# niessner/BundleFusion

Hardware: AMD Instinct MI355X
Metric: frames/sec end-to-end (SIFT+SBA+TSDF re-integrate), 640x480 @4mm (higher is better)
Workload: dtype f32

## Files before the change

### bundlefusion_amd/capi.py

```python
import ctypes as C
import os

import numpy as np

_HERE = os.path.dirname(os.path.abspath(__file__))
LIB_PATH = os.environ.get("BF_LIB_PATH") or os.path.join(_HERE, "lib", "libbf_hip.so")


class BFError(RuntimeError):
    pass


if not os.path.exists(LIB_PATH):
    raise ImportError(
        "bundlefusion_amd: %s is missing — build it with `python -c 'import __graft_entry__ as g; g.build()'` "
        "(there is no CPU fallback)" % LIB_PATH)

try:
    import torch
except ImportError:
    pass
lib = C.CDLL(LIB_PATH, mode=C.RTLD_GLOBAL)

SDF_BLOCK_SIZE = 8
# ... 212 lines not shown
            o.d_texels = None; o.wait_event = None
        check(lib.bf_scene_run_batch(self._h, arr, len(ops), C.byref(cam)))

    def garbage_collect(self):
        check(lib.bf_scene_garbage_collect(self._h))

    def compactify(self, cam_to_world, cam):
        check(lib.bf_scene_set_last_rigid_transform_and_compactify(self._h, mat16(cam_to_world), C.byref(cam)))

    def hash_data(self):
        hd = HashData()
        check(lib.bf_scene_get_hash_data(self._h, C.byref(hd)))
        return hd

    def hash_params(self):
        p = HashParams()
        check(lib.bf_scene_get_hash_params(self._h, C.byref(p)))
        return p

    def heap_free_count(self):
        v = C.c_uint32()
        check(lib.bf_scene_get_heap_free_count(self._h, C.byref(v)))
        return v.value

    def num_allocated_blocks(self):
        v = C.c_uint32()
        check(lib.bf_scene_get_num_allocated_blocks(self._h, C.byref(v)))
        return v.value

    def num_integrated_frames(self):
        v = C.c_uint32()
        check(lib.bf_scene_get_num_integrated_frames(self._h, C.byref(v)))
        return v.value

    def debug_hash(self):
        out = (C.c_uint32 * 6)()
        check(lib.bf_scene_debug_hash(self._h, out))
        return dict(occupied=out[0], heap_free=out[1], duplicate_keys=out[2], free_and_allocated=out[3], leaked=out[4],
                    dropped=out[5])

    def find_blocks(self, pos):
        import torch
        out = torch.empty(pos.shape[0], dtype=torch.int32, device=pos.device)
        check(lib.bf_scene_debug_find_blocks(self._h, C.c_void_p(pos.data_ptr()), int(pos.shape[0]), C.c_void_p(out.data_ptr())))
        return out

    def kernel_timing(self, enable):
        check(lib.bf_scene_kernel_timing(self._h, int(enable)))

    def kernel_timing_read(self):
        n, ms = C.c_uint32(), C.c_float()
        check(lib.bf_scene_kernel_timing_read(self._h, C.byref(n), C.byref(ms)))
        return n.value, ms.value

    def kernel_timing_occupied(self):
        v = C.c_uint64(); n = C.c_uint32()
        check(lib.bf_scene_kernel_timing_occupied(self._h, C.byref(v), C.byref(n)))
        return v.value, n.value

    def kernel_timing_blocks(self):
        a = C.c_uint64(); b = C.c_uint64(); c = C.c_uint64(); n = C.c_uint32()
        check(lib.bf_scene_kernel_timing_blocks(self._h, C.byref(a), C.byref(b), C.byref(c), C.byref(n)))
        return a.value, b.value, c.value, n.value

    def kernel_timing_images(self):
        n = C.c_uint32()
# ... 1233 lines not shown
```

### bundlefusion_amd/csrc/tsdf.hip

```cpp
#include <hip/hip_runtime.h>

#include <algorithm>
#include <cmath>
#include <cstdlib>
#include <cstring>
#include <strings.h>
#include <unordered_map>
#include <unordered_set>
#include <vector>

#include "bf_device.h"
#include "bf_internal.h"
#include "../../include/bf_comm.h"

using namespace bf;

namespace {

constexpr int BS = BF_SDF_BLOCK_SIZE;
constexpr int VOX = BS * BS * BS;
constexpr uint32_t NBINS = 256;
constexpr uint32_t BINCAP = 4096;
constexpr uint32_t OVCAP = 4096;
constexpr uint32_t TILE = 1024;
constexpr uint64_t EMPTY64 = ~0ull;
constexpr int KEYLIM = 1 << 20;

struct AllocRec { uint64_t key; int32_t ptr; uint32_t pad; };
struct BinRec { uint64_t key; uint32_t bucket; uint32_t aux; };

enum Stat { ST_DROPPED = 0, ST_ERROR = 1, ST_STUCK = 2, ST_TICKET = 3, ST_COUNT = 4 };
enum ErrBits { ERR_BIN_OVERFLOW = 1, ERR_DEDUPE_FULL = 2, ERR_OV_OVERFLOW = 4, ERR_GC_MISSING = 8, ERR_LIST_FULL = 16 };

struct Dev {
    bf_hash_entry* hash;
    uint32_t* heap;
    uint32_t* heapCounter;
    bf_voxel* vox;
    bf_hash_entry* compact;
    uint32_t* compactSrc;
    int32_t* compactCount;
    AllocRec* allocList;
    AllocRec* allocListAlt;
    uint32_t* allocCount;
    uint32_t* allocSnap;
    uint64_t* dedupe;
    uint32_t dedupeMask;
    BinRec* bins;
    uint32_t* binCount;
    BinRec* overflow;
    uint32_t* overflowCount;
    uint32_t* stuckSlots;
    uint32_t* tileCounts;
    uint32_t* stats;
    unsigned long long* occSum;
};

struct Frame {
    m44 T, Tinv;
    bf_depth_camera_params cam;
    uint32_t numBuckets;
    uint32_t maxChain;
    uint32_t numSDFBlocks;
    float voxelSize;
// ... 1260 lines not shown
    const uint32_t lane = threadIdx.x & 63u;
    const uint32_t wave = __builtin_amdgcn_readfirstlane(blockIdx.x * 4u + (threadIdx.x >> 6)), nWaves = gridDim.x * 4u;
    if (accumulate && wave == 0 && lane == 0) {
        if (MODE == 2) { d.occSum[2] += (unsigned long long)n; d.occSum[0] += (unsigned long long)(uint32_t)d.compactCount[1]; }
        else { d.occSum[0] += (unsigned long long)n; d.occSum[1] += (unsigned long long)n; }
    }
    if (wave >= n) return;
    const __amdgpu_buffer_rsrc_t texRes = __builtin_amdgcn_make_buffer_rsrc(const_cast<uint2*>(tex), 0, (int)(2u * c.bytes), 0x00020000);
    for (uint32_t blk = wave; blk < n; blk += nWaves) {
        const ApxEntry en = apxEntry<MODE>(d, blk);
        const ApxBlock cur = apxBlock<DE, IN>(d, c, in, de, en.e, en.flags, lane);
#pragma unroll 1
        for (int z = 0; z < 8; z += 2) {
            ApxPair pa;
            apxSamples<DE, IN>(c, in, de, cur, z, texRes, pa);
            bool anyA, anyB;
            apxTouched<DE, IN>(c, pa, anyA, anyB);
            const bool ldA = __builtin_amdgcn_ballot_w64(anyA) != 0ull, ldB = __builtin_amdgcn_ballot_w64(anyB) != 0ull;
            if (!ldA && !ldB) continue;
            apxLoadVoxels(cur, z, pa, ldA, ldB);
            apxStageB<DE, IN, RNE>(c, cur, z, pa);
        }
    }
}


__global__ void k_probe_cvt(uint32_t* out) {
    const float v[8] = {0.5f, 1.5f, 2.5f, 2.7f, 254.4f, 300.0f, -3.0f, 3.49f};
    if (threadIdx.x < 8) out[threadIdx.x] = __builtin_amdgcn_cvt_pk_u8_f32(v[threadIdx.x], 1u, 0xAABBCCDDu);
}

#include "tsdf_batch.h"

__global__ __launch_bounds__(256) void k_gc_identify(Dev d, Frame f, uint32_t needMask) {
    __shared__ uint32_t wmax[4];
    const uint32_t n = (uint32_t)d.compactCount[0];
    for (uint32_t blk = blockIdx.x; blk < n; blk += gridDim.x) {
        if (needMask != 0u && (reinterpret_cast<const uint32_t*>(d.compact)[(size_t)blk * 8 + 4] & needMask) == 0u) continue;
        const int4 e = reinterpret_cast<const int4*>(d.compact)[(size_t)blk * 2];
        const bf_voxel* v = d.vox + (size_t)(uint32_t)e.w;
        const uint32_t w0 = (uint32_t)f2i(v[2 * threadIdx.x + 0].weight);
        const uint32_t w1 = (uint32_t)f2i(v[2 * threadIdx.x + 1].weight);
        uint32_t m = wave_max_u(max(w0, w1));
        if ((threadIdx.x & 63) == 0) wmax[threadIdx.x >> 6] = m;
        __syncthreads();
        if (threadIdx.x == 0) {
            m = max(max(wmax[0], wmax[1]), max(wmax[2], wmax[3]));
            if (m == 0) {
                i3 b; b.x = e.x; b.y = e.y; b.z = e.z;
                const uint32_t h = hashPos(f.numBuckets, b);
                const uint32_t bin = (uint32_t)(((uint64_t)h * NBINS) / f.numBuckets);
                const uint32_t pos = atomicAdd(&d.binCount[bin], 1u);
                if (pos < BINCAP) {
                    BinRec r; r.key = packKey(b); r.bucket = h; r.aux = d.compactSrc[blk];
                    d.bins[(size_t)bin * BINCAP + pos] = r;
                } else {
                    atomicOr(&d.stats[ST_ERROR], (uint32_t)ERR_BIN_OVERFLOW);
                }
            }
        }
        __syncthreads();
    }
}

BF_DEV int32_t deleteEntry(const Dev& d, const Frame& f, i3 b, uint32_t h) {
    const uint32_t hp = h * BF_HASH_BUCKET_SIZE;
    const uint32_t total = BF_HASH_BUCKET_SIZE * f.numBuckets;
    uint4* h4 = reinterpret_cast<uint4*>(d.hash);
    for (uint32_t j = 0; j < BF_HASH_BUCKET_SIZE; ++j) {
        const uint32_t i = hp + j;
        const bf_hash_entry c = d.hash[i];
        if (c.pos[0] == b.x && c.pos[1] == b.y && c.pos[2] == b.z && c.ptr != BF_FREE_ENTRY) {
            if (c.offset != 0) {
                const uint32_t next = (i + c.offset) % total;
                h4[(size_t)i * 2] = h4[(size_t)next * 2];
                h4[(size_t)i * 2 + 1] = h4[(size_t)next * 2 + 1];
                h4[(size_t)next * 2] = make_uint4(0, 0, 0, (uint32_t)BF_FREE_ENTRY);
                h4[(size_t)next * 2 + 1] = make_uint4(0, 0, 0, 0);
            } else {
                h4[(size_t)i * 2] = make_uint4(0, 0, 0, (uint32_t)BF_FREE_ENTRY);
                h4[(size_t)i * 2 + 1] = make_uint4(0, 0, 0, 0);
            }
            return c.ptr;
        }
    }
    const uint32_t last = hp + BF_HASH_BUCKET_SIZE - 1;
    bf_hash_entry c = d.hash[last];
    uint32_t prev = last;
    uint32_t i = (last + c.offset) % total;
    for (uint32_t it = 0; it < f.maxChain; ++it) {
        c = d.hash[i];
        if (c.pos[0] == b.x && c.pos[1] == b.y && c.pos[2] == b.z && c.ptr != BF_FREE_ENTRY) {
            h4[(size_t)i * 2] = make_uint4(0, 0, 0, (uint32_t)BF_FREE_ENTRY);
            h4[(size_t)i * 2 + 1] = make_uint4(0, 0, 0, 0);
            d.hash[prev].offset = c.offset;
            return c.ptr;
        }
        if (c.offset == 0) return BF_FREE_ENTRY;
        prev = i;
        i = (last + c.offset) % total;
    }
    return BF_FREE_ENTRY;
}

__global__ __launch_bounds__(1024) void k_gc_delete(Dev d, Frame f) {
    __shared__ SortLds s;
    __shared__ uint32_t scratch[16];
    const uint32_t bin = blockIdx.x;
    const uint32_t n = min(d.binCount[bin], BINCAP);
    if (n == 0) return;
    loadBinSorted(s, d.bins + (size_t)bin * BINCAP, n);
    const uint32_t base = binPrefix(d.binCount, bin, scratch);
    const uint32_t heapC = d.heapCounter[0];
    for (uint32_t idx = threadIdx.x; idx < n; idx += blockDim.x) {
        const uint32_t h = s.bucket[idx];
        if (idx > 0 && s.bucket[idx - 1] == h) continue;
        for (uint32_t k = idx; k < n && s.bucket[k] == h; ++k) {
            const int32_t ptr = deleteEntry(d, f, unpackKey(s.key[k]), h);
            d.allocList[s.aux[k]].ptr = BF_FREE_ENTRY;
            if (ptr == BF_FREE_ENTRY) { atomicOr(&d.stats[ST_ERROR], (uint32_t)ERR_GC_MISSING); s.aux[k] = 0xFFFFFFFFu; continue; }
            d.heap[heapC + 1u + base + k] = (uint32_t)ptr / (uint32_t)VOX;
            s.aux[k] = (uint32_t)ptr;
        }
    }
    __syncthreads();
    for (uint32_t k = 0; k < n; ++k) {
        const uint32_t ptr = s.aux[k];
        if (ptr == 0xFFFFFFFFu) continue;
        uint4* v4 = reinterpret_cast<uint4*>(d.vox + (size_t)ptr);
        for (uint32_t t = threadIdx.x; t < (uint32_t)(VOX * 12 / 16); t += blockDim.x) v4[t] = make_uint4(0, 0, 0, 0);
    }
}

__global__ __launch_bounds__(256) void k_gc_finish(Dev d) {
    __shared__ uint32_t scratch[16];
    const uint32_t D = binPrefix(d.binCount, NBINS, scratch);
    if (threadIdx.x == 0) d.heapCounter[0] += D;
    __syncthreads();
    for (uint32_t b = threadIdx.x; b < NBINS; b += blockDim.x) d.binCount[b] = 0;
}

}

struct bf_scene {
    bf_hash_params params;
    bf_depth_camera_params cam;
    bool haveCam = false;
    Dev d{};
    hipStream_t stream = nullptr;
    uint32_t numIntegrated = 0;
    uint32_t dedupeSize = 0;
    uint32_t gridCompact = 0, gridUpdateCol = 0, gridUpdateColPlain = 0;
    bool forceExactDiv = false;
    bool externalAlloc = false;
    bf_comm* allocComm = nullptr;
    uint32_t allocCap = 0;
    uint8_t *d_allocSend = nullptr, *d_allocRecv = nullptr; uint32_t* d_allocSlots = nullptr;
    uint8_t *d_batchSend = nullptr, *d_batchRecv = nullptr;
    int arith = BF_TSDF_ARITH_FAST;
    int cvtRne = -1;
    uint2* texel[8] = {}; size_t texelPixels = 0;
    int32_t* d_hashDecision = nullptr;
    uint32_t shardLo = 0, shardHi = 0xFFFFFFFFu;
    uint32_t opsTimed = 0;
    uint32_t imagesTimed = 0;
    bool overlap = false;
    hipStream_t prep = nullptr;
    static constexpr int NBMAX = 8;
    int NB = 4;
    bf_hash_entry* cbuf[NBMAX] = {}; uint32_t* csrc[NBMAX] = {}; int32_t* ccnt[NBMAX] = {};
    int cur = 0;
    hipEvent_t evPrep[NBMAX] = {}, evUpd[NBMAX] = {}, evBarrier = nullptr, evTmp = nullptr;
    bool updRecorded[NBMAX] = {};
    bool barrierPending = false;
    hipEvent_t pendingEv = nullptr;
    const uint2* frameTexels = nullptr;
    bool compactStale = false;
    uint32_t gcMask = 0;
    BatchDev bd{};
    bool batchReady = false;
    uint2* btexel[NBMAX][BF_SCENE_BATCH_MAX] = {}; size_t btexelPixels = 0;
    uint32_t updateLds = 0;
    const char* verifyPath = nullptr; bf_voxel* vshadow[2] = {}; VerifyLog* vlog = nullptr; uint32_t vseq = 0;
    bool timing = false;
    std::vector<std::pair<hipEvent_t, hipEvent_t>> events;
    size_t eventsUsed = 0;
    std::vector<void*> allocations;
};

#define BF_TRY_RC(expr) do { int _rc = (expr); if (_rc != BF_OK) return _rc; } while (0)

namespace {

template <class T>
int devAlloc(bf_scene* s, T** p, size_t count) {
    void* q = nullptr;
    hipError_t e = BF_MALLOC(&q, count * sizeof(T));
    if (e != hipSuccess) { set_error("BF_MALLOC(%zu B) failed: %s", count * sizeof(T), hipGetErrorString(e)); return BF_ERR_HIP; }
    s->allocations.push_back(q);
    *p = (T*)q;
    return BF_OK;
}

Frame makeFrame(const bf_scene* s) {
    Frame f;
    memcpy(f.T.e, s->params.m_rigidTransform, 64);
    memcpy(f.Tinv.e, s->params.m_rigidTransformInverse, 64);
    f.cam = s->cam;
    f.numBuckets = s->params.m_hashNumBuckets;
    f.maxChain = s->params.m_hashMaxCollisionLinkedListSize;
// ... 337 lines not shown
    bc.tile0 = (uint32_t)((uint64_t)tiles * rank / world); bc.tile1 = (uint32_t)((uint64_t)tiles * (rank + 1) / world);
    if (bc.tile1 > bc.tile0) hipLaunchKernelGGL(k_batch_march, dim3(div_up(bc.tile1 - bc.tile0, 4), n), dim3(256), 0, ms, dv, s->bd, bc, ma);
    if (s->allocComm) {
        const uint64_t brec = 8 + sizeof(BatchRec) * (uint64_t)s->allocCap;
        hipLaunchKernelGGL(k_batch_pack, dim3(256), dim3(256), 0, ms, dv, s->bd, reinterpret_cast<uint32_t*>(s->d_batchSend), reinterpret_cast<BatchRec*>(s->d_batchSend + 8), s->allocCap);
        hipLaunchKernelGGL(k_batch_pack_finish, dim3(1), dim3(1), 0, ms, s->bd);
        BF_TRY_RC(bf_comm_all_gather(s->allocComm, s->d_batchSend, s->d_batchRecv, brec, ms));
        for (uint32_t r = 0; r < world; ++r) {
            const uint8_t* base = s->d_batchRecv + brec * r;
            hipLaunchKernelGGL(k_batch_ingest, dim3(256), dim3(256), 0, ms, dv, s->bd, reinterpret_cast<const uint32_t*>(base), reinterpret_cast<const BatchRec*>(base + 8), s->allocCap);
        }
    }
    if (s->overlap && s->barrierPending) { BF_HIP_TRY(hipStreamWaitEvent(ps, s->evBarrier, 0)); s->barrierPending = false; }
    hipLaunchKernelGGL(k_batch_bin, dim3(1024), dim3(256), 0, ps, dv, s->bd, bc);
    hipLaunchKernelGGL(k_batch_place, dim3(PLACE_WGS), dim3(256), 0, ps, dv, s->bd, bc, fr);
    if (s->overlap) {
        BF_HIP_TRY(hipEventRecord(s->evPrep[b], ps));
        BF_HIP_TRY(hipStreamWaitEvent(s->stream, s->evPrep[b], 0));
    }
    std::pair<hipEvent_t, hipEvent_t>* ev = nullptr;
    if (s->timing) {
        if (s->eventsUsed == s->events.size()) {
            hipEvent_t e0, e1;
            BF_HIP_TRY(hipEventCreate(&e0));
            BF_HIP_TRY(hipEventCreate(&e1));
            s->events.push_back({e0, e1});
        }
        ev = &s->events[s->eventsUsed++];
        s->opsTimed += opsCount;
        s->imagesTimed += n;
        BF_HIP_TRY(hipEventRecord(ev->first, s->stream));
    }
    const int acc = s->timing ? 1 : 0;
    if (fast) {
        BatchUpdApxArgs ua;
        memset(&ua, 0, sizeof ua);
        ua.nOps = n;
        for (uint32_t k = 0; k < n; ++k) {
            ua.op[k].in = makeApxPose(fin[k]); ua.op[k].de = makeApxPose(fde[k]);
            ua.op[k].tex = ops[k].d_texels ? reinterpret_cast<const uint2*>(ops[k].d_texels) : texelOf[k];
            if (ops[k].data.d_colorData) ua.liveMask |= 3u << (2u * k);
        }
        const ApxCam ac = makeApxCam(fl);
        auto update = [&](const Dev& dd, int accumulate) {
            if (s->cvtRne) hipLaunchKernelGGL((k_update_batch_apx<true>), dim3(s->gridUpdateCol), dim3(256), s->updateLds, s->stream, dd, ac, ua, accumulate);
            else hipLaunchKernelGGL((k_update_batch_apx<false>), dim3(s->gridUpdateCol), dim3(256), s->updateLds, s->stream, dd, ac, ua, accumulate);
        };
        if (s->verifyPath) {
            BF_TRY_RC(verifyBuffers(s));
            hipLaunchKernelGGL(k_verify_copy, dim3(s->gridUpdateCol), dim3(256), 0, s->stream, dv, s->vshadow[0], s->vshadow[1]);
        }
        update(dv, acc);
        if (s->verifyPath) {
            for (int q = 0; q < 2; ++q) { Dev dq = dv; dq.vox = s->vshadow[q]; update(dq, 0); }
            hipLaunchKernelGGL(k_verify_compare, dim3(s->gridUpdateCol), dim3(256), 0, s->stream, dv, s->vshadow[0], s->vshadow[1], s->vlog, s->vseq++, n, s->gridUpdateCol * 4u);
        }
    } else {
        BatchUpdColArgs ua;
        memset(&ua, 0, sizeof ua);
        ua.nOps = n;
        for (uint32_t k = 0; k < n; ++k) {
            ua.op[k].in = makeUpdPose(fin[k]); ua.op[k].de = makeUpdPose(fde[k]);
            ua.op[k].depth = ops[k].data.d_depthData; ua.op[k].color = reinterpret_cast<const uchar4*>(ops[k].data.d_colorData);
        }
        hipLaunchKernelGGL(k_update_batch_col, dim3(s->gridUpdateCol), dim3(256), 0, s->stream, dv, makeUpdCam(fl), ua, acc, s->forceExactDiv ? 1 : 0);
    }
    if (ev) BF_HIP_TRY(hipEventRecord(ev->second, s->stream));
    if (s->overlap) { BF_HIP_TRY(hipEventRecord(s->evUpd[b], s->stream)); s->updRecorded[b] = true; }
    BF_HIP_TRY(hipGetLastError());
    useBuf(s, b);
    s->compactStale = true;
    s->gcMask = (ops[n - 1].kind == 1 ? 2u : 1u) << (2u * (n - 1));
    for (uint32_t k = 0; k < n; ++k) s->numIntegrated += ops[k].kind == 0 ? 1u : ops[k].kind == 1 ? (uint32_t)-1 : 0u;
    return BF_OK;
}

int checkCall(bf_scene* s, const float* T, const bf_depth_camera_data* data, const bf_depth_camera_params* cam,
              const uint32_t* d_bitMask) {
    BF_REQUIRE(s && T && data && cam, "null argument");
    BF_REQUIRE(data->d_depthData, "d_depthData is null");
    BF_REQUIRE(d_bitMask == nullptr, "chunk streaming (d_bitMask) is not supported: it is disabled for BundleFusion");
    BF_REQUIRE(cam->m_imageWidth > 0 && cam->m_imageHeight > 0, "empty image");
    return BF_OK;
}

}

extern "C" {

int bf_scene_create(const bf_hash_params* p, bf_scene** out) {
    BF_REQUIRE(p && out, "null argument");
    BF_REQUIRE(p->m_hashNumBuckets > 0 && p->m_numSDFBlocks > 0, "empty hash / heap");
    BF_REQUIRE(p->m_hashBucketSize == BF_HASH_BUCKET_SIZE, "m_hashBucketSize must be 4 (HASH_BUCKET_SIZE)");
    BF_REQUIRE(p->m_SDFBlockSize == BF_SDF_BLOCK_SIZE, "m_SDFBlockSize must be 8 (SDF_BLOCK_SIZE)");
    BF_REQUIRE((uint64_t)p->m_hashNumBuckets * BF_HASH_BUCKET_SIZE < 0x7FFFFFFFull, "hash too large for 32-bit slot indices");
    BF_REQUIRE((uint64_t)p->m_numSDFBlocks * VOX < 0x7FFFFFFFull, "too many SDF blocks for the reference's int ptr");
    int ndev = 0;
    if (hipGetDeviceCount(&ndev) != hipSuccess || ndev == 0) { set_error("no HIP device visible"); return BF_ERR_NO_DEVICE; }
    bf_scene* s = new bf_scene();
    s->params = *p;
    const size_t numEntries = (size_t)p->m_hashNumBuckets * BF_HASH_BUCKET_SIZE;
    const size_t N = p->m_numSDFBlocks;
    uint32_t ds = 1u << 16;
    while (ds < 2u * NBINS * BINCAP && ds < 4u * N) ds <<= 1;
    s->dedupeSize = ds;
    int rc = BF_OK;
#define A(ptr, cnt) if (rc == BF_OK) rc = devAlloc(s, &(ptr), (cnt))
    A(s->d.hash, numEntries);
    A(s->d.heap, N);
    A(s->d.heapCounter, 1);
    A(s->d.vox, N * VOX);
    for (int b = 0; b < bf_scene::NBMAX; ++b) { A(s->cbuf[b], N); A(s->csrc[b], N); A(s->ccnt[b], 4); }
    A(s->d.occSum, 3);
    A(s->d.allocList, N);
    A(s->d.allocListAlt, N);
    A(s->d.allocCount, 1);
    A(s->d.dedupe, (size_t)ds);
    A(s->d.bins, (size_t)NBINS * BINCAP);
    A(s->d.binCount, NBINS);
    A(s->d.overflow, OVCAP);
    A(s->d.overflowCount, 1);
    A(s->d.stuckSlots, OVCAP);
    A(s->d.tileCounts, N / TILE + 4);
    A(s->d.stats, ST_COUNT);
    A(s->d_hashDecision, 4);
#undef A
    if (rc != BF_OK) { bf_scene_destroy(s); return rc; }
    s->d.dedupeMask = ds - 1;
    useBuf(s, 0);
    {
        int least = 0, greatest = 0;
        BF_HIP_TRY(hipDeviceGetStreamPriorityRange(&least, &greatest));
        BF_HIP_TRY(hipStreamCreateWithPriority(&s->prep, hipStreamNonBlocking, greatest));
    }
    for (int b = 0; b < bf_scene::NBMAX; ++b)
        for (hipEvent_t* e : {&s->evPrep[b], &s->evUpd[b]}) BF_HIP_TRY(hipEventCreateWithFlags(e, hipEventDisableTiming));
    for (hipEvent_t* e : {&s->evBarrier, &s->evTmp})
        BF_HIP_TRY(hipEventCreateWithFlags(e, hipEventDisableTiming));
    s->gridCompact = std::min<uint32_t>(std::max<uint32_t>(div_up((uint32_t)N, TILE), 1u), 2048u);
    s->gridUpdateCol = s->gridUpdateColPlain = 8192;
    if (const char* e = getenv("BF_TSDF_EXACT_DIV")) s->forceExactDiv = atoi(e) != 0;
    if (const char* e = getenv("BF_DEBUG_VERIFY_BATCH")) s->verifyPath = e;
    if (const char* e = getenv("BF_DEBUG_UPDATE_LDS")) s->updateLds = (uint32_t)atoi(e);
    *out = s;
    int rcReset = bf_scene_reset(s);
    if (rcReset != BF_OK) return rcReset;
    int arith = BF_TSDF_ARITH_FAST;
    if (const char* e = getenv("BF_TSDF_ARITH")) {
        if (strcasecmp(e, "exact") == 0) arith = BF_TSDF_ARITH_EXACT;
        else if (strcasecmp(e, "fast") == 0) arith = BF_TSDF_ARITH_FAST;
        else { set_error("BF_TSDF_ARITH must be 'fast' or 'exact' (got '%s')", e); bf_scene_destroy(s); *out = nullptr; return BF_ERR_INVALID_ARG; }
    }
    return bf_scene_set_arith(s, arith);
}

int bf_scene_set_external_alloc(bf_scene* s, int enable) {
    BF_REQUIRE(s, "null scene");
// ... 207 lines not shown
    setLastRigidTransform(s, newT);
    const Frame f = makeFrame(s);
    return runOperator(s, 2, f, fo, data);
}

int bf_scene_run_batch(bf_scene* s, const bf_scene_batch_op* ops, uint32_t n, const bf_depth_camera_params* cam) {
    BF_REQUIRE(s && ops && cam, "null argument");
    BF_REQUIRE(n >= 1 && n <= BF_SCENE_BATCH_MAX, "1 .. BF_SCENE_BATCH_MAX operators per batch");
    BF_REQUIRE(cam->m_imageWidth > 0 && cam->m_imageHeight > 0, "empty image");
    for (uint32_t k = 0; k < n; ++k) {
        BF_REQUIRE(ops[k].kind >= 0 && ops[k].kind <= 2, "unknown operator kind");
        BF_REQUIRE(ops[k].data.d_depthData, "d_depthData is null");
    }
    s->cam = *cam; s->haveCam = true;
    return runBatch(s, ops, n);
}

int bf_scene_set_last_rigid_transform_and_compactify(bf_scene* s, const float T[16], const bf_depth_camera_params* cam) {
    BF_REQUIRE(s && T && cam, "null argument");
    s->cam = *cam; s->haveCam = true;
    setLastRigidTransform(s, T);
    BF_TRY_RC(beginExclusive(s));
    BF_TRY_RC(launchCompactify(s));
    return endExclusive(s);
}

int bf_scene_garbage_collect(bf_scene* s) {
    BF_REQUIRE(s, "null scene");
    if (!s->haveCam) return BF_OK;
    BF_TRY_RC(beginExclusive(s));
    uint32_t needMask = 0;
    if (s->compactStale) { if (s->gcMask) needMask = s->gcMask; else BF_TRY_RC(launchCompactify(s)); }
    const Frame f = makeFrame(s);
    hipLaunchKernelGGL(k_gc_identify, dim3(4096), dim3(256), 0, s->stream, s->d, f, needMask);
    hipLaunchKernelGGL(k_gc_delete, dim3(NBINS), dim3(1024), 0, s->stream, s->d, f);
    hipLaunchKernelGGL(k_gc_finish, dim3(1), dim3(256), 0, s->stream, s->d);
    hipLaunchKernelGGL(k_compact_count, dim3(s->gridCompact), dim3(256), 0, s->stream, s->d);
    hipLaunchKernelGGL(k_compact_scatter, dim3(s->gridCompact), dim3(256), 0, s->stream, s->d);
    hipLaunchKernelGGL(k_list_commit, dim3(1), dim3(1), 0, s->stream, s->d);
    std::swap(s->d.allocList, s->d.allocListAlt);
    BF_HIP_TRY(hipGetLastError());
    s->compactStale = true; s->gcMask = 0;
    return endExclusive(s);
}

int bf_scene_get_hash_data(bf_scene* s, bf_hash_data* out) {
    BF_REQUIRE(s && out, "null argument");
    BF_TRY_RC(refreshStaleList(s));
    BF_TRY_RC(syncAll(s));
    out->d_heap = s->d.heap;
    out->d_heapCounter = s->d.heapCounter;
    out->d_hashDecision = s->d_hashDecision;
    out->d_hashDecisionPrefix = nullptr;
    out->d_hash = s->d.hash;
    out->d_hashCompactified = s->d.compact;
    out->d_hashCompactifiedCounter = s->d.compactCount;
    out->d_SDFBlocks = s->d.vox;
    out->d_hashBucketMutex = nullptr;
    return BF_OK;
}

static int checkDeviceErrors(bf_scene* s) {
    uint32_t stats[ST_COUNT];
    BF_HIP_TRY(hipMemcpyAsync(stats, s->d.stats, sizeof stats, hipMemcpyDeviceToHost, s->stream));
    BF_HIP_TRY(hipStreamSynchronize(s->stream));
    if (stats[ST_ERROR]) { set_error("TSDF scratch capacity exceeded during an earlier operator (error bits 0x%x: 1 bin, 2 de-dup set, 4 overflow list, 8 GC, 16 block list)", stats[ST_ERROR]); return BF_ERR_CAPACITY; }
    return BF_OK;
}

// ... 12 lines not shown
int bf_scene_get_heap_free_count(bf_scene* s, uint32_t* out) {
    BF_REQUIRE(s && out, "null argument");
    BF_TRY_RC(syncAll(s));
    uint32_t c = 0;
    BF_HIP_TRY(hipMemcpyAsync(&c, s->d.heapCounter, 4, hipMemcpyDeviceToHost, s->stream));
    BF_HIP_TRY(hipStreamSynchronize(s->stream));
    *out = c + 1u;
    return BF_OK;
}

int bf_scene_get_num_integrated_frames(bf_scene* s, uint32_t* out) {
    BF_REQUIRE(s && out, "null argument");
    *out = s->numIntegrated;
    return BF_OK;
}

int bf_scene_set_last_rigid_transform(bf_scene* s, const float camToWorld[16]) {
    BF_REQUIRE(s && camToWorld, "null argument");
    setLastRigidTransform(s, camToWorld);
    return BF_OK;
}

int bf_scene_get_num_allocated_blocks(bf_scene* s, uint32_t* out) {
    BF_REQUIRE(s && out, "null argument");
    BF_TRY_RC(syncAll(s));
    uint32_t n = 0;
    BF_HIP_TRY(hipMemcpyAsync(&n, s->d.allocCount, 4, hipMemcpyDeviceToHost, s->stream));
    BF_HIP_TRY(hipStreamSynchronize(s->stream));
    std::vector<AllocRec> recs(n);
    if (n) BF_HIP_TRY(hipMemcpy(recs.data(), s->d.allocList, (size_t)n * sizeof(AllocRec), hipMemcpyDeviceToHost));
    uint32_t live = 0;
    for (auto& r : recs) live += (r.ptr != BF_FREE_ENTRY);
    *out = live;
    return BF_OK;
}

int bf_scene_debug_hash(bf_scene* s, uint32_t out[6]) {
    BF_REQUIRE(s && out, "null argument");
    BF_TRY_RC(syncAll(s));
    BF_HIP_TRY(hipStreamSynchronize(s->stream));
    const size_t numEntries = (size_t)s->params.m_hashNumBuckets * BF_HASH_BUCKET_SIZE;
    const uint32_t N = s->params.m_numSDFBlocks;
    std::vector<bf_hash_entry> hash(numEntries);
    std::vector<uint32_t> heap(N);
    uint32_t heapCounter = 0, stats[ST_COUNT];
    BF_HIP_TRY(hipMemcpy(hash.data(), s->d.hash, numEntries * sizeof(bf_hash_entry), hipMemcpyDeviceToHost));
    BF_HIP_TRY(hipMemcpy(heap.data(), s->d.heap, (size_t)N * 4, hipMemcpyDeviceToHost));
    BF_HIP_TRY(hipMemcpy(&heapCounter, s->d.heapCounter, 4, hipMemcpyDeviceToHost));
    BF_HIP_TRY(hipMemcpy(stats, s->d.stats, sizeof stats, hipMemcpyDeviceToHost));
    const uint32_t nFree = heapCounter + 1u;
    std::vector<uint8_t> state(N, 0);
    uint32_t dupFree = 0;
    for (uint32_t i = 0; i < nFree && i < N; ++i) { if (state[heap[i]] == 1) dupFree++; state[heap[i]] = 1; }
    uint32_t occupied = 0, both = 0, dupKeys = 0;
    std::unordered_set<uint64_t> keys;
    for (size_t i = 0; i < numEntries; ++i) {
        if (hash[i].ptr == BF_FREE_ENTRY) continue;
        occupied++;
        const uint32_t blk = (uint32_t)hash[i].ptr / VOX;
        if (blk < N) { if (state[blk] == 1) both++; else state[blk] = 2; }
        i3 b; b.x = hash[i].pos[0]; b.y = hash[i].pos[1]; b.z = hash[i].pos[2];
        if (!keys.insert(packKey(b)).second) dupKeys++;
    }
    uint32_t leaked = dupFree;
    for (uint32_t i = 0; i < N; ++i) leaked += (state[i] == 0);
    out[0] = occupied; out[1] = nFree; out[2] = dupKeys; out[3] = both; out[4] = leaked; out[5] = stats[ST_DROPPED];
// ... 80 lines not shown
```

### bundlefusion_amd/csrc/tsdf_batch.h

```cpp

constexpr uint32_t BMAX = BF_SCENE_BATCH_MAX;
static_assert(2 * BMAX <= 32, "two membership bits per operator in the 32-bit flags word of a list entry");
static_assert(BMAX <= 12 && (uint64_t)NBINS * BINCAP <= (1u << 20), "record packing: operator in 4 bits, needing operators in 12, rank among an operator's keys in 20");

struct BatchDev {
    unsigned long long* set; uint32_t setMask;
    uint32_t* opMask;
    uint32_t* candList; uint32_t* candCount; uint32_t candCap;
    BinRec* bins;
    uint32_t* binCount;
    uint32_t* bucketCnt;
    uint32_t* flags;
};

struct BatchCommon {
    bf_depth_camera_params cam;
    uint32_t numBuckets, maxChain, numSDFBlocks;
    float voxelSize, maxIntegrationDistance, truncScale, truncation;
    uint32_t shardLo, shardHi;
    uint32_t nOps;
    uint32_t tile0, tile1;
};
struct alignas(64) BatchMarchOp { m44 T, Tinv; const float* depth; const uint32_t* color; uint2* texel; uint32_t marches; uint32_t pad; };
struct BatchMarchArgs { BatchMarchOp op[BMAX]; };
// ... 430 lines not shown
            batchAppendBlock(d, keepMask(c, fr, r.key, r.ptr, 0u), r.key, r.ptr, i, L.wscan, &L.sbase);
        }
    }
    asm volatile("s_waitcnt vmcnt(0)" ::: "memory");
    __syncthreads();
    if (tid == 0) {
        const uint32_t ticket = atomicAdd(&d.stats[ST_TICKET], 1u);
        L.lastFlag = ticket == gridDim.x - 1 ? 1u : 0u;
        if (L.lastFlag) __builtin_amdgcn_fence(__ATOMIC_ACQUIRE, "agent");
    }
    __syncthreads();
    if (!L.lastFlag) return;
    if (slowMode) batchReplay(d, bd, c, fr, L, heapC0, allocBase0);
    else if (tid == 0) {
        for (uint32_t k = 0; k < nOps; ++k) {
            const uint32_t listRoom = N - min(L.opAllocBase[k], N);
            if (L.opM[k] > listRoom && listRoom < L.opHeapC[k] + 1u) atomicOr(&d.stats[ST_ERROR], (uint32_t)ERR_LIST_FULL);
        }
    }
    if (tid == 0) {
        d.heapCounter[0] = L.opHeapC[nOps];
        d.allocCount[0] = L.opAllocBase[nOps];
        d.allocSnap[0] = L.opAllocBase[nOps];
        d.overflowCount[0] = 0;
        bd.candCount[0] = 0u; bd.flags[0] = 0u;
        d.stats[ST_TICKET] = 0;
    }
    for (uint32_t i = tid; i < nOps * NBINS; i += 256u) bd.binCount[i] = 0u;
    if (fl & 2u)
        for (uint32_t i = tid; i <= bd.setMask; i += 256u) { bd.set[i] = EMPTY64; bd.opMask[i] = 0u; }
}

struct alignas(64) BatchUpdOpApx { ApxPose in, de; const uint2* tex; };
struct BatchUpdApxArgs { BatchUpdOpApx op[BMAX]; uint32_t nOps; uint32_t liveMask; };

#ifdef BF_VAR_VLOAD
struct KargMirrorApx { Dev d; ApxCam c; BatchUpdApxArgs a; int accumulate; };
BF_DEV BatchUpdOpApx loadOpVector(uint32_t k) {
    typedef uint32_t v4u __attribute__((ext_vector_type(4)));
    const uint64_t ka = (uint64_t)__builtin_amdgcn_kernarg_segment_ptr() + offsetof(KargMirrorApx, a) + (uint64_t)k * sizeof(BatchUpdOpApx);
    const volatile v4u* src = reinterpret_cast<const volatile v4u*>(ka);
    union { BatchUpdOpApx o; uint32_t w[sizeof(BatchUpdOpApx) / 4]; } u;
#pragma unroll
    for (uint32_t i = 0; i < sizeof(BatchUpdOpApx) / 16; ++i) {
        const v4u v = src[i];
        u.w[4 * i + 0] = __builtin_amdgcn_readfirstlane(v.x); u.w[4 * i + 1] = __builtin_amdgcn_readfirstlane(v.y);
        u.w[4 * i + 2] = __builtin_amdgcn_readfirstlane(v.z); u.w[4 * i + 3] = __builtin_amdgcn_readfirstlane(v.w);
    }
    return u.o;
}
#endif

template <bool RNE>
__global__ __launch_bounds__(256) void k_update_batch_apx(Dev d, ApxCam c, BatchUpdApxArgs a, int accumulate) {
    const uint32_t n = (uint32_t)d.compactCount[0];
    const uint32_t lane = threadIdx.x & 63u;
    const uint32_t wave = __builtin_amdgcn_readfirstlane(blockIdx.x * 4u + (threadIdx.x >> 6)), nWaves = gridDim.x * 4u;
    if (accumulate && wave == 0 && lane == 0) { d.occSum[2] += (unsigned long long)n; d.occSum[0] += (unsigned long long)(uint32_t)d.compactCount[1]; }
    if (wave >= n) return;
    for (uint32_t blk = wave; blk < n; blk += nWaves) {
        const int4 e = reinterpret_cast<const int4*>(d.compact)[(size_t)blk * 2];
        const uint32_t mask = reinterpret_cast<const uint32_t*>(d.compact)[(size_t)blk * 8 + 4] & a.liveMask;
        if (mask == 0u) continue;
        uint32_t* base = reinterpret_cast<uint32_t*>(d.vox + ((size_t)(uint32_t)e.w + lane));
        v2f vS[4], vW[4]; uint32_t vCA[4], vCB[4];
#pragma unroll
        for (int p = 0; p < 4; ++p) {
            const uint32_t* vpA = base + (size_t)(2 * p) * 64u * 3u; const uint32_t* vpB = vpA + 64u * 3u;
            vS[p].x = __uint_as_float(vpA[0]); vW[p].x = __uint_as_float(vpA[1]); vCA[p] = vpA[2];
            vS[p].y = __uint_as_float(vpB[0]); vW[p].y = __uint_as_float(vpB[1]); vCB[p] = vpB[2];
        }
        uint32_t dirty = 0u;
        for (uint32_t k = 0; k < a.nOps; ++k) {
            const uint32_t m = (mask >> (2u * k)) & 3u;
            if (m == 0u) continue;
#ifdef BF_VAR_VLOAD
            const BatchUpdOpApx o = loadOpVector(k);
#else
            const BatchUpdOpApx& o = a.op[k];
#endif
            const __amdgpu_buffer_rsrc_t texRes = __builtin_amdgcn_make_buffer_rsrc(const_cast<uint2*>(o.tex), 0, (int)(2u * c.bytes), 0x00020000);
            const ApxBlock cur = apxBlock<true, true>(d, c, o.in, o.de, e, m, lane);
#pragma unroll
            for (int pp = 0; pp < 4; ++pp) {
#ifdef BF_VAR_REVERSE_PAIRS
                const int p = 3 - pp;
#else
                const int p = pp;
#endif
                ApxPair pa;
                apxSamples<true, true>(c, o.in, o.de, cur, 2 * p, texRes, pa);
                bool stA, stB;
                apxCompute<true, true, RNE>(c, pa, vS[p], vW[p], vCA[p], vCB[p], stA, stB);
                dirty |= ((stA ? 1u : 0u) << (2 * p)) | ((stB ? 2u : 0u) << (2 * p));
            }
        }
#pragma unroll
        for (int p = 0; p < 4; ++p) {
            uint32_t* vpA = base + (size_t)(2 * p) * 64u * 3u; uint32_t* vpB = vpA + 64u * 3u;
            if (__builtin_amdgcn_ballot_w64((dirty >> (2 * p)) & 1u) != 0ull) { vpA[0] = __float_as_uint(vS[p].x); vpA[1] = __float_as_uint(vW[p].x); vpA[2] = vCA[p]; }
            if (__builtin_amdgcn_ballot_w64((dirty >> (2 * p + 1)) & 1u) != 0ull) { vpB[0] = __float_as_uint(vS[p].y); vpB[1] = __float_as_uint(vW[p].y); vpB[2] = vCB[p]; }
        }
    }
}

struct VerifyRec { uint32_t seq, blk, vox, which; int32_t ex, ey, ez; uint32_t mask; uint32_t val[3][3]; uint32_t nOps, hwWave, pad[5]; };
static_assert(sizeof(VerifyRec) == 96, "record layout (tools/verify_stream.py)");
struct VerifyLog { uint32_t count, cap, batches, blocks; VerifyRec rec[1]; };

__global__ __launch_bounds__(256) void k_verify_copy(Dev d, bf_voxel* s0, bf_voxel* s1) {
    const uint32_t n = (uint32_t)d.compactCount[0];
    const uint32_t lane = threadIdx.x & 63u, wave = blockIdx.x * 4u + (threadIdx.x >> 6), nWaves = gridDim.x * 4u;
    for (uint32_t blk = wave; blk < n; blk += nWaves) {
        const uint32_t ptr = (uint32_t)reinterpret_cast<const int4*>(d.compact)[(size_t)blk * 2].w;
        const uint32_t* src = reinterpret_cast<const uint32_t*>(d.vox + ptr);
        uint32_t* a = reinterpret_cast<uint32_t*>(s0 + ptr); uint32_t* b = reinterpret_cast<uint32_t*>(s1 + ptr);
        for (uint32_t i = lane; i < VOX * 3u; i += 64u) { const uint32_t v = src[i]; a[i] = v; b[i] = v; }
    }
}
__global__ __launch_bounds__(256) void k_verify_compare(Dev d, const bf_voxel* s0, const bf_voxel* s1, VerifyLog* log, uint32_t seq, uint32_t nOps, uint32_t nWavesUpd) {
    const uint32_t n = (uint32_t)d.compactCount[0];
    const uint32_t lane = threadIdx.x & 63u, wave = blockIdx.x * 4u + (threadIdx.x >> 6), nWaves = gridDim.x * 4u;
    if (wave == 0 && lane == 0) { atomicAdd(&log->batches, 1u); atomicAdd(&log->blocks, n); }
    for (uint32_t blk = wave; blk < n; blk += nWaves) {
        const int4 e = reinterpret_cast<const int4*>(d.compact)[(size_t)blk * 2];
        const uint32_t mask = reinterpret_cast<const uint32_t*>(d.compact)[(size_t)blk * 8 + 4];
        const uint32_t* r = reinterpret_cast<const uint32_t*>(d.vox + (uint32_t)e.w);
        const uint32_t* a = reinterpret_cast<const uint32_t*>(s0 + (uint32_t)e.w); const uint32_t* b = reinterpret_cast<const uint32_t*>(s1 + (uint32_t)e.w);
        for (uint32_t v = lane; v < VOX; v += 64u) {
            uint32_t x[3][3];
            for (int q = 0; q < 3; ++q) { x[0][q] = r[v * 3 + q]; x[1][q] = a[v * 3 + q]; x[2][q] = b[v * 3 + q]; }
            const bool d01 = x[0][0] != x[1][0] || x[0][1] != x[1][1] || x[0][2] != x[1][2];
            const bool d02 = x[0][0] != x[2][0] || x[0][1] != x[2][1] || x[0][2] != x[2][2];
            const bool d12 = x[1][0] != x[2][0] || x[1][1] != x[2][1] || x[1][2] != x[2][2];
            if (d01 || d02 || d12) {
                const uint32_t pos = atomicAdd(&log->count, 1u);
                if (pos < log->cap) {
                    VerifyRec& o = log->rec[pos];
                    o.seq = seq; o.blk = blk; o.vox = v; o.which = (d01 ? 1u : 0u) | (d02 ? 2u : 0u) | (d12 ? 4u : 0u);
                    o.ex = e.x; o.ey = e.y; o.ez = e.z; o.mask = mask; o.nOps = nOps; o.hwWave = blk % nWavesUpd;
                    for (int c = 0; c < 3; ++c) for (int q = 0; q < 3; ++q) o.val[c][q] = x[c][q];
                }
            }
        }
    }
}

struct alignas(64) BatchUpdOpCol { UpdPose in; float padIn[2]; UpdPose de; float padDe[2]; const float* depth; const uchar4* color; };
struct BatchUpdColArgs { BatchUpdOpCol op[BMAX]; uint32_t nOps; uint32_t pad; };

__global__ __launch_bounds__(256) void k_update_batch_col(Dev d, UpdCam c, BatchUpdColArgs a, int accumulate, int forceExact) {
    const uint32_t n = (uint32_t)d.compactCount[0];
    const uint32_t lane = threadIdx.x & 63u;
    const uint32_t wave = blockIdx.x * 4u + (threadIdx.x >> 6), nWaves = gridDim.x * 4u;
    if (accumulate && wave == 0 && lane == 0) { d.occSum[2] += (unsigned long long)n; d.occSum[0] += (unsigned long long)(uint32_t)d.compactCount[1]; }
    for (uint32_t blk = wave; blk < n; blk += nWaves) {
        const int4 e = reinterpret_cast<const int4*>(d.compact)[(size_t)blk * 2];
        const uint32_t mask = reinterpret_cast<const uint32_t*>(d.compact)[(size_t)blk * 8 + 4];
        for (uint32_t k = 0; k < a.nOps; ++k) {
            const uint32_t m = (mask >> (2u * k)) & 3u;
            const BatchUpdOpCol& o = a.op[k];
            if (m == 0u || o.color == nullptr) continue;
            bool fast = !forceExact;
            if (m & 2u) fast = fast && blockFast(c, o.de, e);
            if (m & 1u) fast = fast && blockFast(c, o.in, e);
            if (fast) colFast<true, true>(d, c, o.in, o.de, e, m, lane, o.depth, reinterpret_cast<const uint32_t*>(o.color));
            else colExact<true, true>(d, c, o.in, o.de, e, m, lane, o.depth, o.color);
        }
    }
}
```

### include/bf_hip.h

```cpp
#ifndef BF_HIP_H
#define BF_HIP_H

#include <stddef.h>
#include <stdint.h>

#ifdef __cplusplus
extern "C" {
#endif

#define BF_API __attribute__((visibility("default")))

typedef enum bf_status {
    BF_OK = 0,
    BF_ERR_INVALID_ARG = -1,
    BF_ERR_HIP = -2,
    BF_ERR_NO_DEVICE = -3,
    BF_ERR_CAPACITY = -4,
    BF_ERR_STATE = -5,
    BF_ERR_NOT_ON_DEVICE = -6
} bf_status;

BF_API const char* bf_last_error(void);
BF_API const char* bf_version(void);
BF_API int bf_device_count(void);
// ... 86 lines not shown
BF_API int bf_scene_set_external_alloc(bf_scene* s, int enable);
BF_API int bf_scene_alloc_collect(bf_scene* s, const float cam_to_world[16], const bf_depth_camera_data* data, const bf_depth_camera_params* cam,
                                  uint32_t part, uint32_t parts, uint64_t* d_keys, uint32_t* d_slots, uint32_t* d_count, uint32_t capacity);
BF_API int bf_scene_alloc_ingest(bf_scene* s, const uint64_t* d_keys, const uint32_t* d_count, uint32_t capacity);
BF_API int bf_scene_alloc_place(bf_scene* s);
BF_API int bf_scene_alloc_sync(bf_scene* s);
#define BF_TSDF_ARITH_EXACT 0
#define BF_TSDF_ARITH_FAST 1
BF_API int bf_scene_set_arith(bf_scene* s, int mode);
BF_API int bf_scene_set_frame_texels(bf_scene* s, const void* d_texels);
BF_API int bf_image_interleave_texels(void* d_texels, const float* d_depth, const uint8_t* d_colorRGBX, uint32_t numPixels, void* hip_stream);
BF_API int bf_scene_get_arith(bf_scene* s, int* mode);
BF_API int bf_scene_reintegrate(bf_scene* s, const float old_cam_to_world[16], const float new_cam_to_world[16],
                                const bf_depth_camera_data* data, const bf_depth_camera_params* cam);
#define BF_SCENE_BATCH_MAX 12
typedef struct bf_scene_batch_op {
    int32_t kind;
    int32_t reserved;
    float T0[16], T1[16];
    bf_depth_camera_data data;
    const void* d_texels;
    void* wait_event;
} bf_scene_batch_op;
BF_API int bf_scene_run_batch(bf_scene* s, const bf_scene_batch_op* ops, uint32_t n, const bf_depth_camera_params* cam);
BF_API int bf_scene_garbage_collect(bf_scene* s);
BF_API int bf_scene_set_last_rigid_transform_and_compactify(
    bf_scene* s, const float cam_to_world[16], const bf_depth_camera_params* cam);
BF_API int bf_scene_set_last_rigid_transform(bf_scene* s, const float cam_to_world[16]);
BF_API int bf_scene_get_hash_data(bf_scene* s, bf_hash_data* out);
BF_API int bf_scene_get_hash_params(bf_scene* s, bf_hash_params* out);
BF_API int bf_scene_get_heap_free_count(bf_scene* s, uint32_t* out);
BF_API int bf_scene_get_num_integrated_frames(bf_scene* s, uint32_t* out);
BF_API int bf_scene_debug_hash(bf_scene* s, uint32_t out[6]);
BF_API int bf_scene_debug_find_blocks(bf_scene* s, const int32_t* d_pos, uint32_t n, int32_t* d_ptr_out);
BF_API int bf_scene_get_num_allocated_blocks(bf_scene* s, uint32_t* out);
BF_API int bf_scene_kernel_timing(bf_scene* s, int enable);
BF_API int bf_scene_kernel_timing_read(bf_scene* s, uint32_t* count, float* total_ms);
BF_API int bf_scene_kernel_timing_occupied(bf_scene* s, uint64_t* sumOccupiedBlocks, uint32_t* numOps);
BF_API int bf_scene_kernel_timing_images(bf_scene* s, uint32_t* numImages);
BF_API int bf_scene_kernel_timing_blocks(bf_scene* s, uint64_t* sumOperatorBlocks, uint64_t* visitedPlain, uint64_t* visitedFused, uint32_t* numOps);



typedef struct bf_cached_frame {
    float* d_depthDownsampled;
    float* d_cameraposDownsampled;
    float* d_intensityDownsampled;
    float* d_intensityDerivsDownsampled;
    uint8_t* d_normalsDownsampledUCHAR4;
    float* d_normalsDownsampled;
} bf_cached_frame;

typedef struct bf_cache bf_cache;

BF_API int bf_cache_create(uint32_t widthDepthInput, uint32_t heightDepthInput, uint32_t widthDownSampled,
                           uint32_t heightDownSampled, uint32_t maxNumImages, const float inputIntrinsics[16],
                           float colorDownSigma, float depthDownSigmaD, float depthDownSigmaR, bf_cache** out);
BF_API int bf_cache_destroy(bf_cache* c);
BF_API int bf_cache_set_stream(bf_cache* c, void* hip_stream);
BF_API int bf_cache_store_frame(bf_cache* c, const float* d_depth, uint32_t inputDepthWidth, uint32_t inputDepthHeight,
                                const uint8_t* d_color, uint32_t inputColorWidth, uint32_t inputColorHeight);
BF_API int bf_cache_reset(bf_cache* c);
BF_API int bf_cache_copy_cache_frame_from(bf_cache* c, bf_cache* other, uint32_t frameFrom);
BF_API int bf_cache_increment(bf_cache* c);
BF_API int bf_cache_get_num_frames(bf_cache* c, uint32_t* out);
BF_API int bf_cache_set_current_frame(bf_cache* c, uint32_t n);
// ... 267 lines not shown
```

Measured before the change: 1330.

## Fold GC zero-weight detection into batch update kernels and triage GC work

The batch update kernels now compute, for blocks touched by the last op, whether any voxel weight is nonzero and record a known/nonzero flag in the compact entry. A new triage kernel uses these flags to bin empty blocks directly and compacts only the undecided blocks into a work list, so the identify kernel rereads voxel weights only for those. The delete kernel's voxel zeroing is also flattened across all deleted blocks for better thread utilisation. This adds a wave reduction and a store per block in the update path, plus an extra kernel launch and work buffer, and it depends on the flag word in the compact entry being valid.

```diff
diff --git a/bundlefusion_amd/capi.py b/bundlefusion_amd/capi.py
--- a/bundlefusion_amd/capi.py
+++ b/bundlefusion_amd/capi.py
@@ -268,6 +268,11 @@
         v = C.c_uint32()
         check(lib.bf_scene_get_num_integrated_frames(self._h, C.byref(v)))
         return v.value
+
+    def gc_stats(self):
+        out = (C.c_uint32 * 2)()
+        check(lib.bf_scene_get_gc_stats(self._h, out))
+        return dict(from_update=out[0], from_voxels=out[1])
 
     def debug_hash(self):
         out = (C.c_uint32 * 6)()
diff --git a/bundlefusion_amd/csrc/tsdf.hip b/bundlefusion_amd/csrc/tsdf.hip
--- a/bundlefusion_amd/csrc/tsdf.hip
+++ b/bundlefusion_amd/csrc/tsdf.hip
@@ -29,7 +29,10 @@
 struct AllocRec { uint64_t key; int32_t ptr; uint32_t pad; };
 struct BinRec { uint64_t key; uint32_t bucket; uint32_t aux; };
 
-enum Stat { ST_DROPPED = 0, ST_ERROR = 1, ST_STUCK = 2, ST_TICKET = 3, ST_COUNT = 4 };
+enum Stat { ST_DROPPED = 0, ST_ERROR = 1, ST_STUCK = 2, ST_TICKET = 3,
+            ST_GC_WORK = 4, ST_GC_ACC = 5,
+            ST_GC_UPD = 6, ST_GC_VOX = 7,
+            ST_COUNT = 8 };
 enum ErrBits { ERR_BIN_OVERFLOW = 1, ERR_DEDUPE_FULL = 2, ERR_OV_OVERFLOW = 4, ERR_GC_MISSING = 8, ERR_LIST_FULL = 16 };
 
 struct Dev {
@@ -1356,11 +1359,49 @@
 
 #include "tsdf_batch.h"
 
-__global__ __launch_bounds__(256) void k_gc_identify(Dev d, Frame f, uint32_t needMask) {
+BF_DEV void gcBinZero(const Dev& d, const Frame& f, int4 e, uint32_t blk) {
+    i3 b; b.x = e.x; b.y = e.y; b.z = e.z;
+    const uint32_t h = hashPos(f.numBuckets, b);
+    const uint32_t bin = (uint32_t)(((uint64_t)h * NBINS) / f.numBuckets);
+    const uint32_t pos = atomicAdd(&d.binCount[bin], 1u);
+    if (pos < BINCAP) {
+        BinRec r; r.key = packKey(b); r.bucket = h; r.aux = d.compactSrc[blk];
+        d.bins[(size_t)bin * BINCAP + pos] = r;
+    } else {
+        atomicOr(&d.stats[ST_ERROR], (uint32_t)ERR_BIN_OVERFLOW);
+    }
+}
+
+__global__ __launch_bounds__(256) void k_gc_triage(Dev d, Frame f, uint32_t needMask, uint32_t* __restrict__ work) {
+    const uint32_t n = (uint32_t)d.compactCount[0];
+    const uint32_t lane = threadIdx.x & 63u;
+    uint32_t decided = 0u;
+    for (uint32_t base = blockIdx.x * 256u; base < n; base += gridDim.x * 256u) {
+        const uint32_t blk = base + threadIdx.x;
+        uint2 w = make_uint2(0u, 0u);
+        if (blk < n) w = reinterpret_cast<const uint2*>(d.compact)[(size_t)blk * 4 + 2];
+        const bool need = (w.x & needMask) != 0u, known = (w.y & GC_KNOWN) != 0u;
+        if (need && known) {
+            decided++;
+            if ((w.y & GC_NONZERO) == 0u) gcBinZero(d, f, reinterpret_cast<const int4*>(d.compact)[(size_t)blk * 2], blk);
+        }
+        const unsigned long long um = __builtin_amdgcn_ballot_w64(need && !known);
+        if (um != 0ull) {
+            uint32_t at = 0u;
+            if (lane == 0u) at = atomicAdd(&d.stats[ST_GC_WORK], (uint32_t)__popcll(um));
+            at = __shfl(at, 0, 64);
+            if (need && !known) work[at + (uint32_t)__popcll(um & ((1ull << lane) - 1ull))] = blk;
+        }
+    }
+    decided = (uint32_t)wave_sum_i((int)decided);
+    if (lane == 0u && decided != 0u) atomicAdd(&d.stats[ST_GC_ACC], decided);
+}
+
+__global__ __launch_bounds__(256) void k_gc_identify(Dev d, Frame f, const uint32_t* __restrict__ work) {
     __shared__ uint32_t wmax[4];
-    const uint32_t n = (uint32_t)d.compactCount[0];
-    for (uint32_t blk = blockIdx.x; blk < n; blk += gridDim.x) {
-        if (needMask != 0u && (reinterpret_cast<const uint32_t*>(d.compact)[(size_t)blk * 8 + 4] & needMask) == 0u) continue;
+    const uint32_t n = work ? d.stats[ST_GC_WORK] : (uint32_t)d.compactCount[0];
+    for (uint32_t i = blockIdx.x; i < n; i += gridDim.x) {
+        const uint32_t blk = work ? work[i] : i;
         const int4 e = reinterpret_cast<const int4*>(d.compact)[(size_t)blk * 2];
         const bf_voxel* v = d.vox + (size_t)(uint32_t)e.w;
         const uint32_t w0 = (uint32_t)f2i(v[2 * threadIdx.x + 0].weight);
@@ -1370,18 +1411,7 @@
         __syncthreads();
         if (threadIdx.x == 0) {
             m = max(max(wmax[0], wmax[1]), max(wmax[2], wmax[3]));
-            if (m == 0) {
-                i3 b; b.x = e.x; b.y = e.y; b.z = e.z;
-                const uint32_t h = hashPos(f.numBuckets, b);
-                const uint32_t bin = (uint32_t)(((uint64_t)h * NBINS) / f.numBuckets);
-                const uint32_t pos = atomicAdd(&d.binCount[bin], 1u);
-                if (pos < BINCAP) {
-                    BinRec r; r.key = packKey(b); r.bucket = h; r.aux = d.compactSrc[blk];
-                    d.bins[(size_t)bin * BINCAP + pos] = r;
-                } else {
-                    atomicOr(&d.stats[ST_ERROR], (uint32_t)ERR_BIN_OVERFLOW);
-                }
-            }
+            if (m == 0) gcBinZero(d, f, e, blk);
         }
         __syncthreads();
     }
@@ -1448,18 +1478,23 @@
         }
     }
     __syncthreads();
-    for (uint32_t k = 0; k < n; ++k) {
-        const uint32_t ptr = s.aux[k];
+    constexpr uint32_t PIECES = (uint32_t)(VOX * 12 / 16);
+    for (uint32_t i = threadIdx.x; i < n * PIECES; i += blockDim.x) {
+        const uint32_t k = i / PIECES, ptr = s.aux[k];
         if (ptr == 0xFFFFFFFFu) continue;
-        uint4* v4 = reinterpret_cast<uint4*>(d.vox + (size_t)ptr);
-        for (uint32_t t = threadIdx.x; t < (uint32_t)(VOX * 12 / 16); t += blockDim.x) v4[t] = make_uint4(0, 0, 0, 0);
-    }
-}
-
-__global__ __launch_bounds__(256) void k_gc_finish(Dev d) {
+        reinterpret_cast<uint4*>(d.vox + (size_t)ptr)[i - k * PIECES] = make_uint4(0, 0, 0, 0);
+    }
+}
+
+__global__ __launch_bounds__(256) void k_gc_finish(Dev d, int triaged) {
     __shared__ uint32_t scratch[16];
     const uint32_t D = binPrefix(d.binCount, NBINS, scratch);
-    if (threadIdx.x == 0) d.heapCounter[0] += D;
+    if (threadIdx.x == 0) {
+        d.heapCounter[0] += D;
+        d.stats[ST_GC_UPD] = d.stats[ST_GC_ACC];
+        d.stats[ST_GC_VOX] = triaged ? d.stats[ST_GC_WORK] : (uint32_t)d.compactCount[0];
+        d.stats[ST_GC_ACC] = 0u; d.stats[ST_GC_WORK] = 0u;
+    }
     __syncthreads();
     for (uint32_t b = threadIdx.x; b < NBINS; b += blockDim.x) d.binCount[b] = 0;
 }
@@ -1500,6 +1535,7 @@
     hipEvent_t pendingEv = nullptr;
     const uint2* frameTexels = nullptr;
     bool compactStale = false;
+    uint32_t* gcWork = nullptr;
     uint32_t gcMask = 0;
     BatchDev bd{};
     bool batchReady = false;
@@ -1903,10 +1939,12 @@
         BF_HIP_TRY(hipEventRecord(ev->first, s->stream));
     }
     const int acc = s->timing ? 1 : 0;
+    const uint32_t gcBit = (ops[n - 1].kind == 1 ? 2u : 1u) << (2u * (n - 1));
     if (fast) {
         BatchUpdApxArgs ua;
         memset(&ua, 0, sizeof ua);
         ua.nOps = n;
+        ua.gcBit = gcBit;
         for (uint32_t k = 0; k < n; ++k) {
             ua.op[k].in = makeApxPose(fin[k]); ua.op[k].de = makeApxPose(fde[k]);
             ua.op[k].tex = ops[k].d_texels ? reinterpret_cast<const uint2*>(ops[k].d_texels) : texelOf[k];
@@ -1930,6 +1968,7 @@
         BatchUpdColArgs ua;
         memset(&ua, 0, sizeof ua);
         ua.nOps = n;
+        ua.gcBit = gcBit;
         for (uint32_t k = 0; k < n; ++k) {
             ua.op[k].in = makeUpdPose(fin[k]); ua.op[k].de = makeUpdPose(fde[k]);
             ua.op[k].depth = ops[k].data.d_depthData; ua.op[k].color = reinterpret_cast<const uchar4*>(ops[k].data.d_colorData);
@@ -1941,7 +1980,7 @@
     BF_HIP_TRY(hipGetLastError());
     useBuf(s, b);
     s->compactStale = true;
-    s->gcMask = (ops[n - 1].kind == 1 ? 2u : 1u) << (2u * (n - 1));
+    s->gcMask = gcBit;
     for (uint32_t k = 0; k < n; ++k) s->numIntegrated += ops[k].kind == 0 ? 1u : ops[k].kind == 1 ? (uint32_t)-1 : 0u;
     return BF_OK;
 }
@@ -1994,6 +2033,7 @@
     A(s->d.stuckSlots, OVCAP);
     A(s->d.tileCounts, N / TILE + 4);
     A(s->d.stats, ST_COUNT);
+    A(s->gcWork, N);
     A(s->d_hashDecision, 4);
 #undef A
     if (rc != BF_OK) { bf_scene_destroy(s); return rc; }
@@ -2267,9 +2307,10 @@
     uint32_t needMask = 0;
     if (s->compactStale) { if (s->gcMask) needMask = s->gcMask; else BF_TRY_RC(launchCompactify(s)); }
     const Frame f = makeFrame(s);
-    hipLaunchKernelGGL(k_gc_identify, dim3(4096), dim3(256), 0, s->stream, s->d, f, needMask);
+    if (needMask) hipLaunchKernelGGL(k_gc_triage, dim3(256), dim3(256), 0, s->stream, s->d, f, needMask, s->gcWork);
+    hipLaunchKernelGGL(k_gc_identify, dim3(4096), dim3(256), 0, s->stream, s->d, f, needMask ? s->gcWork : (const uint32_t*)nullptr);
     hipLaunchKernelGGL(k_gc_delete, dim3(NBINS), dim3(1024), 0, s->stream, s->d, f);
-    hipLaunchKernelGGL(k_gc_finish, dim3(1), dim3(256), 0, s->stream, s->d);
+    hipLaunchKernelGGL(k_gc_finish, dim3(1), dim3(256), 0, s->stream, s->d, needMask ? 1 : 0);
     hipLaunchKernelGGL(k_compact_count, dim3(s->gridCompact), dim3(256), 0, s->stream, s->d);
     hipLaunchKernelGGL(k_compact_scatter, dim3(s->gridCompact), dim3(256), 0, s->stream, s->d);
     hipLaunchKernelGGL(k_list_commit, dim3(1), dim3(1), 0, s->stream, s->d);
@@ -2348,6 +2389,16 @@
     uint32_t live = 0;
     for (auto& r : recs) live += (r.ptr != BF_FREE_ENTRY);
     *out = live;
+    return BF_OK;
+}
+
+int bf_scene_get_gc_stats(bf_scene* s, uint32_t out[2]) {
+    BF_REQUIRE(s && out, "null argument");
+    BF_TRY_RC(syncAll(s));
+    BF_HIP_TRY(hipStreamSynchronize(s->stream));
+    uint32_t stats[ST_COUNT];
+    BF_HIP_TRY(hipMemcpy(stats, s->d.stats, sizeof stats, hipMemcpyDeviceToHost));
+    out[0] = stats[ST_GC_UPD]; out[1] = stats[ST_GC_VOX];
     return BF_OK;
 }
 
diff --git a/bundlefusion_amd/csrc/tsdf_batch.h b/bundlefusion_amd/csrc/tsdf_batch.h
--- a/bundlefusion_amd/csrc/tsdf_batch.h
+++ b/bundlefusion_amd/csrc/tsdf_batch.h
@@ -486,7 +486,9 @@
 }
 
 struct alignas(64) BatchUpdOpApx { ApxPose in, de; const uint2* tex; };
-struct BatchUpdApxArgs { BatchUpdOpApx op[BMAX]; uint32_t nOps; uint32_t liveMask; };
+struct BatchUpdApxArgs { BatchUpdOpApx op[BMAX]; uint32_t nOps; uint32_t liveMask; uint32_t gcBit; };
+
+constexpr uint32_t GC_KNOWN = 1u, GC_NONZERO = 2u;
 
 #ifdef BF_VAR_VLOAD
 struct KargMirrorApx { Dev d; ApxCam c; BatchUpdApxArgs a; int accumulate; };
@@ -514,7 +516,7 @@
     if (wave >= n) return;
     for (uint32_t blk = wave; blk < n; blk += nWaves) {
         const int4 e = reinterpret_cast<const int4*>(d.compact)[(size_t)blk * 2];
-        const uint32_t mask = reinterpret_cast<const uint32_t*>(d.compact)[(size_t)blk * 8 + 4] & a.liveMask;
+        const uint32_t flags = reinterpret_cast<const uint32_t*>(d.compact)[(size_t)blk * 8 + 4], mask = flags & a.liveMask;
         if (mask == 0u) continue;
         uint32_t* base = reinterpret_cast<uint32_t*>(d.vox + ((size_t)(uint32_t)e.w + lane));
         v2f vS[4], vW[4]; uint32_t vCA[4], vCB[4];
@@ -548,6 +550,13 @@
                 apxCompute<true, true, RNE>(c, pa, vS[p], vW[p], vCA[p], vCB[p], stA, stB);
                 dirty |= ((stA ? 1u : 0u) << (2 * p)) | ((stB ? 2u : 0u) << (2 * p));
             }
+        }
+        if (flags & a.gcBit) {
+            uint32_t mw = 0u;
+#pragma unroll
+            for (int p = 0; p < 4; ++p) mw = max(mw, max((uint32_t)f2i(vW[p].x), (uint32_t)f2i(vW[p].y)));
+            mw = wave_max_u(mw);
+            if (lane == 0u) reinterpret_cast<uint32_t*>(d.compact)[(size_t)blk * 8 + 5] = GC_KNOWN | (mw != 0u ? GC_NONZERO : 0u);
         }
 #pragma unroll
         for (int p = 0; p < 4; ++p) {
@@ -601,7 +610,7 @@
 }
 
 struct alignas(64) BatchUpdOpCol { UpdPose in; float padIn[2]; UpdPose de; float padDe[2]; const float* depth; const uchar4* color; };
-struct BatchUpdColArgs { BatchUpdOpCol op[BMAX]; uint32_t nOps; uint32_t pad; };
+struct BatchUpdColArgs { BatchUpdOpCol op[BMAX]; uint32_t nOps; uint32_t gcBit; };
 
 __global__ __launch_bounds__(256) void k_update_batch_col(Dev d, UpdCam c, BatchUpdColArgs a, int accumulate, int forceExact) {
     const uint32_t n = (uint32_t)d.compactCount[0];
@@ -611,15 +620,25 @@
     for (uint32_t blk = wave; blk < n; blk += nWaves) {
         const int4 e = reinterpret_cast<const int4*>(d.compact)[(size_t)blk * 2];
         const uint32_t mask = reinterpret_cast<const uint32_t*>(d.compact)[(size_t)blk * 8 + 4];
+        bool ran = false;
         for (uint32_t k = 0; k < a.nOps; ++k) {
             const uint32_t m = (mask >> (2u * k)) & 3u;
             const BatchUpdOpCol& o = a.op[k];
             if (m == 0u || o.color == nullptr) continue;
+            ran = true;
             bool fast = !forceExact;
             if (m & 2u) fast = fast && blockFast(c, o.de, e);
             if (m & 1u) fast = fast && blockFast(c, o.in, e);
             if (fast) colFast<true, true>(d, c, o.in, o.de, e, m, lane, o.depth, reinterpret_cast<const uint32_t*>(o.color));
             else colExact<true, true>(d, c, o.in, o.de, e, m, lane, o.depth, o.color);
         }
-    }
-}
+        if (ran && (mask & a.gcBit)) {
+            const uint32_t* wp = reinterpret_cast<const uint32_t*>(d.vox + ((size_t)(uint32_t)e.w + lane)) + 1;
+            uint32_t mw = 0u;
+#pragma unroll
+            for (int lz = 0; lz < 8; ++lz) mw = max(mw, (uint32_t)f2i(__uint_as_float(wp[(size_t)lz * 64u * 3u])));
+            mw = wave_max_u(mw);
+            if (lane == 0u) reinterpret_cast<uint32_t*>(d.compact)[(size_t)blk * 8 + 5] = GC_KNOWN | (mw != 0u ? GC_NONZERO : 0u);
+        }
+    }
+}
diff --git a/include/bf_hip.h b/include/bf_hip.h
--- a/include/bf_hip.h
+++ b/include/bf_hip.h
@@ -142,6 +142,7 @@
 BF_API int bf_scene_get_heap_free_count(bf_scene* s, uint32_t* out);
 BF_API int bf_scene_get_num_integrated_frames(bf_scene* s, uint32_t* out);
 BF_API int bf_scene_debug_hash(bf_scene* s, uint32_t out[6]);
+BF_API int bf_scene_get_gc_stats(bf_scene* s, uint32_t out[2]);
 BF_API int bf_scene_debug_find_blocks(bf_scene* s, const int32_t* d_pos, uint32_t n, int32_t* d_ptr_out);
 BF_API int bf_scene_get_num_allocated_blocks(bf_scene* s, uint32_t* out);
 BF_API int bf_scene_kernel_timing(bf_scene* s, int enable);
```

New measurement: 1343 (median of 6 runs). No clear change (+1.0%).
